# ErlerPhilipp/points2surf

Hardware: NVIDIA H100
Metric: SDF queries/sec at grid_res=256 (higher is better)
Workload: dtype f16 operands / f32 accumulate (wgmma); hi/lo split f16 (fp32-level) for FC tails and guard-band recompute

## Files before the change

points2surf_b200/csrc/net_tc.cu:

```cuda
#include "model.cuh"
#include "tc_ptx.cuh"

namespace p2s {

using namespace ptx;

namespace {

constexpr int kTile = 64;
constexpr int kWG = 2;
constexpr int kThreads = 128 * kWG;
template <bool PRECISE>
struct Cfg {
    static constexpr int kChunks = PRECISE ? 2 : 4;
    static constexpr int kSplit = 8 / kChunks;
    static constexpr uint32_t kChunkBytes = PRECISE ? 65536u : 32768u;
    static constexpr uint32_t kW3Bytes = kChunks * kChunkBytes;
    static constexpr uint32_t kMidScale = PRECISE ? 2u : 1u;
    static constexpr uint32_t kMidBytes = (8192u + 8192u + 16384u) * kMidScale;
    static constexpr uint32_t kPerqBytes = PRECISE ? 16384u : 8192u;
    static constexpr uint32_t kRedBytes = 4u * kChunks * 128u * 4u;
    static constexpr uint32_t kOffMid = kW3Bytes;
    static constexpr uint32_t kWgWq = kPerqBytes;
    static constexpr uint32_t kWgBytes = kWgWq + 192 * 4;
    static constexpr uint32_t kOffWg = kOffMid + kMidBytes;
    static constexpr uint32_t kOffBias = kOffWg + kWG * kWgBytes;
    static constexpr uint32_t kSmemBytes = kOffBias + 320 * 4;
};
static_assert(Cfg<false>::kSmemBytes <= 232448 && Cfg<true>::kSmemBytes <= 232448, "shared memory budget");
static_assert(Cfg<false>::kRedBytes <= Cfg<false>::kPerqBytes && Cfg<true>::kRedBytes <= Cfg<true>::kPerqBytes, "reduction scratch");

struct Seg {
    const float* ptr;
    int n;
    int tiles;
    int center;
};

struct PassParams {
    Seg seg[2];
    const float* query;
    const float* R;
    int tiles_per_query;
    int B;
    const float* W0;
    const float* b0;
    int num_mid;
    int mid_N[3];
    const uint8_t* mid_img[3];
    const float* mid_bias[3];
    int perq_layer;
    const uint8_t* perq_img;
    const uint8_t* w3_img;
    float* out;
};

__device__ __forceinline__ uint32_t pack_relu(float a, float b) {
    uint32_t r;
    asm("cvt.rn.relu.satfinite.f16x2.f32 %0, %1, %2;" : "=r"(r) : "f"(b), "f"(a));
    return r;
}
__device__ __forceinline__ void pack_relu_split(float a, float b, uint32_t& hi, uint32_t& lo) {
    hi = pack_relu(a, b);
    const float2 hf = __half22float2(*reinterpret_cast<const __half2*>(&hi));
    lo = pack_half2(fmaxf(a, 0.f) - hf.x, fmaxf(b, 0.f) - hf.y);
}
template <bool PRECISE>
__device__ __forceinline__ void pack_act(float a, float b, uint32_t& hi, uint32_t& lo) {
    if (PRECISE) pack_relu_split(a, b, hi, lo);
    else hi = pack_relu(a, b);
}

template <bool PRECISE, int R>
__device__ __forceinline__ void mid_mma(float (&d)[R], const uint32_t (&a)[4], const uint32_t (&al)[4], uint64_t w, uint64_t w_lo, uint32_t acc) {
    if (R == 32) {
        auto& d32 = reinterpret_cast<float (&)[32]>(d);
        if (PRECISE) { wgmma_rs_n64(d32, al, w, acc); wgmma_rs_n64(d32, a, w_lo, 1); wgmma_rs_n64(d32, a, w, 1); }
        else wgmma_rs_n64(d32, a, w, acc);
    } else {
        auto& d64 = reinterpret_cast<float (&)[64]>(d);
        if (PRECISE) { wgmma_rs_n128(d64, al, w, acc); wgmma_rs_n128(d64, a, w_lo, 1); wgmma_rs_n128(d64, a, w, 1); }
        else wgmma_rs_n128(d64, a, w, acc);
    }
}

template <bool PRECISE, int R, int KL>
__device__ __forceinline__ void pack_acc(const float (&d)[R], const float* bias, int q4, uint32_t (&a)[R / 8][4], uint32_t (&al)[R / 8][KL]) {
#pragma unroll
    for (int j = 0; j < R / 4; ++j) {
        const float2 bb = *reinterpret_cast<const float2*>(bias + 8 * j + 2 * q4);
        pack_act<PRECISE>(d[4 * j] + bb.x, d[4 * j + 1] + bb.y, a[j >> 1][(j & 1) * 2], al[j >> 1][PRECISE ? (j & 1) * 2 : 0]);
        pack_act<PRECISE>(d[4 * j + 2] + bb.x, d[4 * j + 3] + bb.y, a[j >> 1][(j & 1) * 2 + 1], al[j >> 1][PRECISE ? (j & 1) * 2 + 1 : 0]);
    }
}

template <int S>
__device__ __forceinline__ void max_halve(float (&m)[32], int lane) {
    const bool up = (lane & S) != 0;
#pragma unroll
    for (int i = 0; i < S; ++i) {
        const float send = up ? m[i] : m[i + S], keep = up ? m[i + S] : m[i];
        m[i] = fmaxf(keep, __shfl_xor_sync(0xffffffffu, send, S));
    }
}

template <bool PRECISE>
__global__ void __launch_bounds__(kThreads, 1) pointnet_pass_kernel(const PassParams p) {
    using C = Cfg<PRECISE>;
    constexpr int kL = PRECISE ? 4 : 1;
    extern __shared__ __align__(1024) uint8_t smem[];
    float* s_bias = reinterpret_cast<float*>(smem + C::kOffBias);
    const int tid = threadIdx.x, wg = tid >> 7, t = tid & 127, lane = tid & 31, q4 = lane & 3;
    const int r0 = (t >> 5) * 16 + (lane >> 2);
    const int part = blockIdx.x % C::kSplit;
    const int stream = blockIdx.x / C::kSplit, nstreams = gridDim.x / C::kSplit;
    const int nq = (p.B > stream) ? (p.B - stream + nstreams - 1) / nstreams : 0;
    const int tpq = p.tiles_per_query;
    uint32_t mid_off[3] = {0, 0, 0};
    {
        uint32_t o = 0;
        for (int l = 0; l < p.num_mid; ++l) { mid_off[l] = o; o += (uint32_t)p.mid_N[l] * 128u * C::kMidScale; }
    }

    if (nq > 0) {
        const uint4* src = reinterpret_cast<const uint4*>(p.w3_img + (size_t)part * C::kW3Bytes);
        uint4* dst = reinterpret_cast<uint4*>(smem);
        for (uint32_t i = tid; i < C::kW3Bytes / 16; i += kThreads) dst[i] = src[i];
        for (int l = 0; l < p.num_mid; ++l) {
            if (l == p.perq_layer) continue;
            const uint4* s = reinterpret_cast<const uint4*>(p.mid_img[l]);
            uint4* d = reinterpret_cast<uint4*>(smem + C::kOffMid + mid_off[l]);
            for (uint32_t i = tid; i < (uint32_t)p.mid_N[l] * 8u * C::kMidScale; i += kThreads) d[i] = s[i];
        }
    }
    {
        int off = 0;
        for (int l = 0; l < p.num_mid; ++l) {
            for (int i = tid; i < p.mid_N[l]; i += kThreads) s_bias[off + i] = p.mid_bias[l][i];
            off += p.mid_N[l];
        }
        for (int i = tid; i < 64; i += kThreads) s_bias[256 + i] = p.b0[i];
    }
    fence_proxy_async_smem();
    __syncthreads();

    uint8_t* wsm = smem + C::kOffWg + wg * C::kWgBytes;
    uint8_t* perq = wsm;
    float* red = reinterpret_cast<float*>(perq);
    float* wq = reinterpret_cast<float*>(wsm + C::kWgWq);
    const float* s_b0 = s_bias + 256;
    const uint32_t bar_id = 1 + (uint32_t)wg;
    auto wg_sync = [&]() { asm volatile("bar.sync %0, 128;" ::"r"(bar_id) : "memory"); };
    const uint64_t dsc_w3 = make_smem_desc(smem_u32(smem), 128, 2048);
    uint64_t dsc_mid[3], dsc_mid_lo[3];
    for (int l = 0; l < 3; ++l) {
        const bool pq = l == p.perq_layer;
        dsc_mid[l] = make_smem_desc(pq ? smem_u32(perq) : smem_u32(smem + C::kOffMid) + mid_off[l], 128, 1024);
        dsc_mid_lo[l] = dsc_mid[l] + (uint64_t)((pq ? 8192u : (uint32_t)p.mid_N[l] * 128u) >> 4);
    }

    for (int qi = wg; qi < nq; qi += kWG) {
        const size_t q = (size_t)stream + (size_t)qi * nstreams;
        wg_sync();
        if (t < 64) {
            const float w0 = p.W0[t * 3 + 0], w1 = p.W0[t * 3 + 1], w2 = p.W0[t * 3 + 2];
            float r[9] = {1.f, 0.f, 0.f, 0.f, 1.f, 0.f, 0.f, 0.f, 1.f};
            if (p.R) {
#pragma unroll
                for (int i = 0; i < 9; ++i) r[i] = p.R[q * 9 + i];
            }
            wq[0 * 64 + t] = w0 * r[0] + w1 * r[3] + w2 * r[6];
            wq[1 * 64 + t] = w0 * r[1] + w1 * r[4] + w2 * r[7];
            wq[2 * 64 + t] = w0 * r[2] + w1 * r[5] + w2 * r[8];
        }
        if (p.perq_layer >= 0) {
            const uint4* s = reinterpret_cast<const uint4*>(p.perq_img + q * C::kPerqBytes);
            uint4* d = reinterpret_cast<uint4*>(perq);
            for (uint32_t i = t; i < C::kPerqBytes / 16; i += 128) d[i] = s[i];
            fence_proxy_async_smem();
        }
        wg_sync();
        float vmax[4 * C::kChunks];
#pragma unroll
        for (int i = 0; i < 4 * C::kChunks; ++i) vmax[i] = -INFINITY;
        for (int tq = 0; tq < tpq; ++tq) {
            const int sgi = tq < p.seg[0].tiles ? 0 : 1;
            const Seg& sg = p.seg[sgi];
            float cx = 0.f, cy = 0.f, cz = 0.f;
            if (sg.center) { cx = p.query[q * 3 + 0]; cy = p.query[q * 3 + 1]; cz = p.query[q * 3 + 2]; }
            float px[2], py[2], pz[2];
#pragma unroll
            for (int h = 0; h < 2; ++h) {
                int local = (tq - (sgi ? p.seg[0].tiles : 0)) * kTile + r0 + 8 * h;
                if (local >= sg.n) local = 0;
                const float* src = sg.ptr + (q * sg.n + local) * 3;
                px[h] = src[0] - cx; py[h] = src[1] - cy; pz[h] = src[2] - cz;
            }
            uint32_t a[4][4], al[4][kL];
#pragma unroll
            for (int kk = 0; kk < 4; ++kk) {
#pragma unroll
                for (int hc = 0; hc < 2; ++hc) {
                    const int ch = kk * 16 + hc * 8 + 2 * q4;
                    const float2 wx = *reinterpret_cast<const float2*>(wq + 0 * 64 + ch);
                    const float2 wy = *reinterpret_cast<const float2*>(wq + 1 * 64 + ch);
                    const float2 wz = *reinterpret_cast<const float2*>(wq + 2 * 64 + ch);
                    const float2 bb = *reinterpret_cast<const float2*>(s_b0 + ch);
#pragma unroll
                    for (int h = 0; h < 2; ++h) {
                        const float v0 = fmaf(wx.x, px[h], fmaf(wy.x, py[h], fmaf(wz.x, pz[h], bb.x)));
                        const float v1 = fmaf(wx.y, px[h], fmaf(wy.y, py[h], fmaf(wz.y, pz[h], bb.y)));
                        pack_act<PRECISE>(v0, v1, a[kk][hc * 2 + h], al[kk][PRECISE ? hc * 2 + h : 0]);
                    }
                }
            }
            const float* bl = s_bias;
#pragma unroll
            for (int l = 0; l < 2; ++l) {
                if (l >= p.num_mid - 1) break;
                float d[32];
#pragma unroll
                for (int i = 0; i < 32; ++i) d[i] = 0.f;
                wgmma_fence();
#pragma unroll
                for (int ks = 0; ks < 4; ++ks)
                    mid_mma<PRECISE>(d, a[ks], reinterpret_cast<const uint32_t (&)[4]>(al[PRECISE ? ks : 0]), dsc_mid[l] + (uint64_t)(ks * 16), dsc_mid_lo[l] + (uint64_t)(ks * 16), ks > 0);
                wgmma_commit();
                wgmma_wait<0>();
                fence_regs(d);
                pack_acc<PRECISE>(d, bl, q4, a, al);
                bl += 64;
            }
            uint32_t a2[8][4], a2l[8][kL];
            {
                const uint64_t w = p.num_mid == 3 ? dsc_mid[2] : dsc_mid[0], w_lo = p.num_mid == 3 ? dsc_mid_lo[2] : dsc_mid_lo[0];
                float d[64];
#pragma unroll
                for (int i = 0; i < 64; ++i) d[i] = 0.f;
                wgmma_fence();
#pragma unroll
                for (int ks = 0; ks < 4; ++ks)
                    mid_mma<PRECISE>(d, a[ks], reinterpret_cast<const uint32_t (&)[4]>(al[PRECISE ? ks : 0]), w + (uint64_t)(ks * 16), w_lo + (uint64_t)(ks * 16), ks > 0);
                wgmma_commit();
                wgmma_wait<0>();
                fence_regs(d);
                pack_acc<PRECISE>(d, bl, q4, a2, a2l);
            }
#pragma unroll(PRECISE ? 1 : C::kChunks)
            for (int c = 0; c < C::kChunks; ++c) {
                float d[64];
#pragma unroll
                for (int i = 0; i < 64; ++i) d[i] = 0.f;
                const uint64_t w = dsc_w3 + (uint64_t)((uint32_t)c * (C::kChunkBytes >> 4));
                wgmma_fence();
#pragma unroll
                for (int ks = 0; ks < 8; ++ks) {
                    const uint64_t o = w + (uint64_t)(ks * 16);
                    if (PRECISE) {
                        wgmma_rs_n128(d, a2[ks], o + (uint64_t)(32768u >> 4), ks > 0);
                        wgmma_rs_n128(d, reinterpret_cast<const uint32_t (&)[4]>(a2l[PRECISE ? ks : 0]), o, 1);
                        wgmma_rs_n128(d, a2[ks], o, 1);
                    } else {
                        wgmma_rs_n128(d, a2[ks], o, ks > 0);
                    }
                }
                wgmma_commit();
                wgmma_wait<0>();
                fence_regs(d);
                float m[32];
#pragma unroll
                for (int j = 0; j < 16; ++j) {
                    m[2 * j] = fmaxf(d[4 * j], d[4 * j + 2]);
                    m[2 * j + 1] = fmaxf(d[4 * j + 1], d[4 * j + 3]);
                }
                max_halve<16>(m, lane);
                max_halve<8>(m, lane);
                max_halve<4>(m, lane);
                float v[4];
#pragma unroll
                for (int i = 0; i < 4; ++i) v[i] = fmaxf(vmax[i], m[i]);
#pragma unroll
                for (int i = 0; i < 4 * (C::kChunks - 1); ++i) vmax[i] = vmax[i + 4];
#pragma unroll
                for (int i = 0; i < 4; ++i) vmax[4 * (C::kChunks - 1) + i] = v[i];
            }
        }
        constexpr int kC = C::kChunks * 128;
        const int warp = t >> 5;
        wg_sync();
#pragma unroll
        for (int c = 0; c < C::kChunks; ++c)
#pragma unroll
            for (int h = 0; h < 2; ++h)
                *reinterpret_cast<float2*>(red + warp * kC + c * 128 + 16 * (lane >> 2) + 8 * h + 2 * q4) = make_float2(vmax[4 * c + 2 * h], vmax[4 * c + 2 * h + 1]);
        wg_sync();
        for (int i = t; i < kC / 4; i += 128) {
            const float4* r4 = reinterpret_cast<const float4*>(red);
            float4 v = r4[i];
#pragma unroll
            for (int w = 1; w < 4; ++w) {
                const float4 u = r4[w * (kC / 4) + i];
                v = make_float4(fmaxf(v.x, u.x), fmaxf(v.y, u.y), fmaxf(v.z, u.z), fmaxf(v.w, u.w));
            }
            *reinterpret_cast<float4*>(p.out + q * 1024 + (size_t)(part * kC + 4 * i)) = v;
        }
    }
}

__global__ void pack_kmajor_kernel(const float* __restrict__ W, int rows, int K, int row0, uint32_t sbo, uint8_t* __restrict__ img, int lo) {
    int e = blockIdx.x * blockDim.x + threadIdx.x;
    if (e >= rows * K) return;
    int r = e / K, k = e % K;
    uint32_t off = (uint32_t)(r >> 3) * sbo + (uint32_t)(k >> 3) * 128u + (uint32_t)(r & 7) * 16u + (uint32_t)(k & 7) * 2u;
    const float w = W[(size_t)(row0 + r) * K + k];
    const __half h = __float2half_rn(w);
    *reinterpret_cast<__half*>(img + off) = lo ? __float2half_rn(w - __half2float(h)) : h;
}

__global__ void pack_perq_kernel(const float* __restrict__ W, int64_t B, uint8_t* __restrict__ img) {
    int64_t e = (int64_t)blockIdx.x * blockDim.x + threadIdx.x;
    if (e >= B * 4096) return;
    int64_t b = e >> 12;
    int r = (int)((e >> 6) & 63), k = (int)(e & 63);
    uint32_t off = (uint32_t)(r >> 3) * 1024u + (uint32_t)(k >> 3) * 128u + (uint32_t)(r & 7) * 16u + (uint32_t)(k & 7) * 2u;
    *reinterpret_cast<__half*>(img + b * 8192 + off) = __float2half_rn(W[e]);
}

__global__ void __launch_bounds__(256) fold_w1_kernel(const float* __restrict__ W1, const float* __restrict__ T, int64_t B, uint8_t* __restrict__ img) {
    __shared__ float sW[64][65];
    __shared__ __align__(16) float sT[64][68];
    const int64_t b = blockIdx.x;
    const int tid = threadIdx.x;
    for (int e = tid; e < 4096; e += 256) {
        const int r = e >> 6, c = e & 63;
        sW[r][c] = W1[e];
        sT[r][c] = T[b * 4096 + e] + (r == c ? 1.0f : 0.0f);
    }
    __syncthreads();
    const int o = tid >> 2, i0 = (tid & 3) * 16;
    float acc[16];
#pragma unroll
    for (int i = 0; i < 16; ++i) acc[i] = 0.f;
    for (int j = 0; j < 64; ++j) {
        const float w = sW[o][j];
#pragma unroll
        for (int i4 = 0; i4 < 4; ++i4) {
            const float4 t4 = *reinterpret_cast<const float4*>(&sT[j][i0 + 4 * i4]);
            acc[4 * i4 + 0] = fmaf(w, t4.x, acc[4 * i4 + 0]);
            acc[4 * i4 + 1] = fmaf(w, t4.y, acc[4 * i4 + 1]);
            acc[4 * i4 + 2] = fmaf(w, t4.z, acc[4 * i4 + 2]);
            acc[4 * i4 + 3] = fmaf(w, t4.w, acc[4 * i4 + 3]);
        }
    }
    uint8_t* dst = img + b * 8192 + (uint32_t)(o >> 3) * 1024u + (uint32_t)(o & 7) * 16u;
#pragma unroll
    for (int h = 0; h < 2; ++h) {
        uint32_t v[4];
#pragma unroll
        for (int e = 0; e < 4; ++e) v[e] = pack_half2(acc[h * 8 + 2 * e], acc[h * 8 + 2 * e + 1]);
        *reinterpret_cast<uint4*>(dst + (uint32_t)(i0 / 8 + h) * 128u) = make_uint4(v[0], v[1], v[2], v[3]);
    }
}

__global__ void fold_fc3_kernel(const float* __restrict__ W1, const float* __restrict__ Wfc3, const float* __restrict__ bfc3,
                                float* __restrict__ G, float* __restrict__ g0) {
    const int oi = blockIdx.x;
    const int o = oi >> 6, i = oi & 63;
    const int k = threadIdx.x;
    float acc = 0.f;
    for (int j = 0; j < 64; ++j) acc = fmaf(W1[o * 64 + j], Wfc3[(size_t)(j * 64 + i) * 256 + k], acc);
    G[(size_t)oi * 256 + k] = acc;
    if (k == 0) {
        float b = W1[o * 64 + i];
        for (int j = 0; j < 64; ++j) b = fmaf(W1[o * 64 + j], bfc3[j * 64 + i], b);
        g0[oi] = b;
    }
}

__global__ void transpose64_kernel(const float* __restrict__ in, float* __restrict__ out, int64_t B) {
    int64_t e = (int64_t)blockIdx.x * blockDim.x + threadIdx.x;
    if (e >= B * 4096) return;
    int64_t b = e >> 12;
    int i = (int)((e >> 6) & 63), j = (int)(e & 63);
    out[e] = in[b * 4096 + j * 64 + i];
}

__global__ void guard_flag_kernel(const float* __restrict__ logits, int od, int64_t B, float band, int32_t* __restrict__ list, int* __restrict__ count, int64_t base, int64_t cap) {
    int64_t i = (int64_t)blockIdx.x * blockDim.x + threadIdx.x;
    if (i >= B) return;
    if (fabsf(logits[i * od + od - 1]) < band) {
        int slot = atomicAdd(count, 1);
        if (slot < cap) list[slot] = (int32_t)(base + i);
    }
}
__global__ void guard_gather_kernel(const float* __restrict__ src, const int32_t* __restrict__ list, int n, int row_floats, float* __restrict__ dst) {
    int64_t e = (int64_t)blockIdx.x * blockDim.x + threadIdx.x;
    if (e >= (int64_t)n * row_floats) return;
    int i = (int)(e / row_floats), j = (int)(e % row_floats);
    dst[e] = src[(int64_t)list[i] * row_floats + j];
}
__global__ void guard_scatter_kernel(const float* __restrict__ src, const int32_t* __restrict__ list, int n, int od, float* __restrict__ logits) {
    int i = blockIdx.x * blockDim.x + threadIdx.x;
    if (i >= n) return;
    for (int j = 0; j < od; ++j) logits[(int64_t)list[i] * od + j] = src[i * od + j];
}
__global__ void guard_scatter_rows_kernel(const float* __restrict__ src, const int32_t* __restrict__ list, int n, int row_floats, float* __restrict__ dst) {
    int64_t e = (int64_t)blockIdx.x * blockDim.x + threadIdx.x;
    if (e >= (int64_t)n * row_floats) return;
    int i = (int)(e / row_floats), j = (int)(e % row_floats);
    dst[(int64_t)list[i] * row_floats + j] = src[e];
}

}

struct TcStack {
    uint8_t* w3_img = nullptr;
    uint8_t* mid_img[3] = {nullptr, nullptr, nullptr};
    uint8_t* w3_img_p = nullptr;
    uint8_t* mid_img_p[3] = {nullptr, nullptr, nullptr};
    const float* mid_bias[3] = {nullptr, nullptr, nullptr};
    int mid_N[3] = {0, 0, 0};
    int num_mid = 0;
    const float* W0 = nullptr;
    const float* b0 = nullptr;
    const float* b3 = nullptr;
};

struct TcFc {
    const Layer* L = nullptr;
    const uint8_t* img = nullptr;
};
struct TcStnFc { TcFc fc1, fc2, fc3; };

struct TcWeights {
    TcStack qstn;
    TcStack stn[2], fin[2];
    TcStnFc qstn_fc, stn_fc[2];
    TcFc head_fc1[2], head_fc2, head_fc3;
    const uint8_t* fold_img[2] = {nullptr, nullptr};
    const float* fold_bias[2] = {nullptr, nullptr};
    TcStack stn_enc, fin_enc;
    TcStnFc stn_fc_enc;
    TcFc head_fc1_enc;
    const uint8_t* fold_img_enc = nullptr;
    const float* fold_bias_enc = nullptr;
    bool fc_on_tc = true;
    std::vector<void*> allocs;
    int sm_count = 132;
    bool prof_on = false;
    std::vector<std::pair<cudaEvent_t, cudaEvent_t>> prof_events;
    double prof_flops = 0.0;
    ~TcWeights() {
        for (void* a : allocs) cudaFree(a);
        for (auto& e : prof_events) { cudaEventDestroy(e.first); cudaEventDestroy(e.second); }
    }
};

namespace {

uint8_t* tc_alloc(TcWeights& t, size_t bytes) {
    void* p = nullptr;
    P2S_CUDA(cudaMalloc(&p, bytes));
    P2S_CUDA(cudaMemset(p, 0, bytes));
    t.allocs.push_back(p);
    return (uint8_t*)p;
}

uint8_t* pack_layer(TcWeights& t, const Layer& L, uint32_t sbo, bool split = false) {
    const size_t one = (size_t)L.cout * L.cin * 2;
    uint8_t* img = tc_alloc(t, one * (split ? 2 : 1));
    P2S_LAUNCH(pack_kmajor_kernel, (unsigned)cdiv((int64_t)L.cout * L.cin, 256), 256, 0, 0, L.W, L.cout, L.cin, 0, sbo, img, 0);
    if (split) P2S_LAUNCH(pack_kmajor_kernel, (unsigned)cdiv((int64_t)L.cout * L.cin, 256), 256, 0, 0, L.W, L.cout, L.cin, 0, sbo, img + one, 1);
    return img;
}

uint8_t* pack_w3(TcWeights& t, const Layer& L, bool split = false) {
    P2S_CHECK(L.cout == 1024 && L.cin == 128, "big layer must be 128 -> 1024");
    const size_t chunk = split ? 65536 : 32768;
    uint8_t* img = tc_alloc(t, 8 * chunk);
    for (int c = 0; c < 8; ++c) {
        P2S_LAUNCH(pack_kmajor_kernel, (unsigned)cdiv(128 * 128, 256), 256, 0, 0, L.W, 128, 128, c * 128, 2048u, img + (size_t)c * chunk, 0);
        if (split) P2S_LAUNCH(pack_kmajor_kernel, (unsigned)cdiv(128 * 128, 256), 256, 0, 0, L.W, 128, 128, c * 128, 2048u, img + (size_t)c * chunk + 32768, 1);
    }
    return img;
}

void launch_pass(Model& m, const TcStack& s, const Seg& s0, const Seg& s1, const float* query, const float* R,
                 int64_t B, int perq_layer, const uint8_t* perq_img, float* out, cudaStream_t st, bool precise) {
    PassParams p{};
    p.seg[0] = s0; p.seg[1] = s1;
    p.query = query; p.R = R;
    p.tiles_per_query = s0.tiles + s1.tiles;
    p.B = (int)B;
    p.W0 = s.W0; p.b0 = s.b0;
    p.num_mid = s.num_mid;
    for (int l = 0; l < 3; ++l) { p.mid_N[l] = s.mid_N[l]; p.mid_img[l] = precise ? s.mid_img_p[l] : s.mid_img[l]; p.mid_bias[l] = s.mid_bias[l]; }
    p.perq_layer = perq_layer;
    p.perq_img = perq_img;
    p.w3_img = precise ? s.w3_img_p : s.w3_img;
    p.out = out;
    for (int l = 0; l < s.num_mid; ++l)
        P2S_CHECK(s.mid_N[l] == (l == s.num_mid - 1 ? 128 : 64), "pass kernel: mid layers must be 64 -> 64 ... -> 128");
    TcWeights& t = *m.tc;
    const int split = precise ? Cfg<true>::kSplit : Cfg<false>::kSplit;
    int streams = t.sm_count / split;
    if ((int64_t)streams > B) streams = (int)B;
    const int grid = streams * split;
    cudaEvent_t e0 = nullptr, e1 = nullptr;
    const bool prof = t.prof_on && !precise;
    if (prof) {
        P2S_CUDA(cudaEventCreate(&e0)); P2S_CUDA(cudaEventCreate(&e1));
        P2S_CUDA(cudaEventRecord(e0, st));
    }
    if (precise) P2S_LAUNCH(pointnet_pass_kernel<true>, grid, kThreads, Cfg<true>::kSmemBytes, st, p);
    else P2S_LAUNCH(pointnet_pass_kernel<false>, grid, kThreads, Cfg<false>::kSmemBytes, st, p);
    if (prof) {
        P2S_CUDA(cudaEventRecord(e1, st));
        t.prof_events.emplace_back(e0, e1);
        double mac_pt = 3.0 * 64 + 128.0 * 1024;
        int prev = 64;
        for (int l = 0; l < s.num_mid; ++l) { mac_pt += (double)prev * s.mid_N[l]; prev = s.mid_N[l]; }
        t.prof_flops += 2.0 * mac_pt * (double)(s0.n + s1.n) * (double)B;
    }
}

Seg make_seg(const float* ptr, int n, int center) { return Seg{ptr, n, n > 0 ? (n + kTile - 1) / kTile : 0, center}; }

void run_fc(const TcFc& f, const float* in, int lda, float* out, int ldc, int64_t Bc, bool relu, bool on_tc, cudaStream_t st,
            const float* in_bias = nullptr, bool in_relu = false) {
    const Layer& L = *f.L;
    if (on_tc && f.img) launch_fc_tc(in, lda, f.img, L.b, out, ldc, Bc, L.cout, L.cin, relu, st, 0, in_bias, in_relu);
    else {
        P2S_CHECK(!in_bias, "input bias needs the tensor-core FC kernel");
        launch_gemm_nt(in, 0, lda, L.W, 0, L.b, out, 0, ldc, (int)Bc, L.cout, L.cin, 1, relu, st);
    }
}

void fc_tail(const Layer& b3src, const TcStnFc& s, bool on_tc, const float* gmax_raw, int64_t Bc, float* g, float* f1, float* f2, float* out, cudaStream_t st) {
    if (on_tc && s.fc1.img) run_fc(s.fc1, gmax_raw, 1024, f1, 512, Bc, true, true, st, b3src.b, true);
    else {
        P2S_CUDA(cudaMemcpyAsync(g, gmax_raw, (size_t)Bc * 1024 * 4, cudaMemcpyDeviceToDevice, st));
        launch_bias_act(g, b3src.b, Bc, 1024, true, st);
        run_fc(s.fc1, g, 1024, f1, 512, Bc, true, on_tc, st);
    }
    run_fc(s.fc2, f1, 512, f2, 256, Bc, true, on_tc, st);
    run_fc(s.fc3, f2, 256, out, s.fc3.L->cout, Bc, false, on_tc, st);
}

}

void tc_build(Model& m) {
    P2S_CHECK(m.cfg.net_size == 1024, "tensor-core path needs net_size 1024");
    TcWeights* t = new TcWeights();
    m.tc = t;
    cudaDeviceProp prop;
    P2S_CUDA(cudaGetDeviceProperties(&prop, m.device));
    t->sm_count = prop.multiProcessorCount;
    P2S_CUDA(cudaFuncSetAttribute(pointnet_pass_kernel<false>, cudaFuncAttributeMaxDynamicSharedMemorySize, (int)Cfg<false>::kSmemBytes));
    P2S_CUDA(cudaFuncSetAttribute(pointnet_pass_kernel<true>, cudaFuncAttributeMaxDynamicSharedMemorySize, (int)Cfg<true>::kSmemBytes));
    auto build_stn = [&](TcStack& s, const Stn& stn, const Layer* c0a, const Layer* c0b) {
        if (!c0a) {
            s.W0 = stn.c1.W; s.b0 = stn.c1.b;
            s.num_mid = 1;
            s.mid_img[0] = pack_layer(*t, stn.c2, 1024); s.mid_bias[0] = stn.c2.b; s.mid_N[0] = 128;
            s.mid_img_p[0] = pack_layer(*t, stn.c2, 1024, true);
        } else {
            s.W0 = c0a->W; s.b0 = c0a->b;
            s.num_mid = 3;
            s.mid_img[0] = pack_layer(*t, *c0b, 1024); s.mid_bias[0] = c0b->b; s.mid_N[0] = 64;
            s.mid_img[1] = pack_layer(*t, stn.c1, 1024); s.mid_bias[1] = stn.c1.b; s.mid_N[1] = 64;
            s.mid_img[2] = pack_layer(*t, stn.c2, 1024); s.mid_bias[2] = stn.c2.b; s.mid_N[2] = 128;
            s.mid_img_p[0] = pack_layer(*t, *c0b, 1024, true);
            s.mid_img_p[1] = pack_layer(*t, stn.c1, 1024, true);
            s.mid_img_p[2] = pack_layer(*t, stn.c2, 1024, true);
        }
        s.w3_img_p = pack_w3(*t, stn.c3, true);
        s.w3_img = pack_w3(*t, stn.c3);
        s.b3 = stn.c3.b;
    };
    auto build_fin = [&](TcStack& s, const Feat& f) {
        s.W0 = f.conv0a.W; s.b0 = f.conv0a.b;
        s.num_mid = 3;
        s.mid_img[0] = pack_layer(*t, f.conv0b, 1024); s.mid_bias[0] = f.conv0b.b; s.mid_N[0] = 64;
        s.mid_img[1] = nullptr; s.mid_bias[1] = f.conv1.b; s.mid_N[1] = 64;
        s.mid_img[2] = pack_layer(*t, f.conv2, 1024); s.mid_bias[2] = f.conv2.b; s.mid_N[2] = 128;
        s.mid_img_p[0] = pack_layer(*t, f.conv0b, 1024, true);
        s.mid_img_p[2] = pack_layer(*t, f.conv2, 1024, true);
        s.w3_img_p = pack_w3(*t, f.conv3, true);
        s.w3_img = pack_w3(*t, f.conv3);
        s.b3 = f.conv3.b;
    };
    fc_tc_init();
    t->fc_on_tc = !env_flag("P2S_FC_FP32");
    auto mk_fc = [&](const Layer& L) {
        TcFc f;
        f.L = &L;
        f.img = fc_tc_supported(L.cout, L.cin) ? fc_tc_pack(L, t->allocs) : nullptr;
        return f;
    };
    auto mk_stn_fc = [&](const Stn& s) { TcStnFc r; r.fc1 = mk_fc(s.fc1); r.fc2 = mk_fc(s.fc2); r.fc3 = mk_fc(s.fc3); return r; };
    auto fold = [&](const Feat& f, const uint8_t*& img, const float*& bias) {
        P2S_CHECK(f.stn2.fc3.cout == 4096 && f.stn2.fc3.cin == 256 && f.conv1.cout == 64 && f.conv1.cin == 64, "unexpected STN shape");
        float* G = reinterpret_cast<float*>(tc_alloc(*t, (size_t)4096 * 256 * 4));
        float* g0 = reinterpret_cast<float*>(tc_alloc(*t, 4096 * 4));
        P2S_LAUNCH(fold_fc3_kernel, 4096, 256, 0, 0, f.conv1.W, f.stn2.fc3.W, f.stn2.fc3.b, G, g0);
        img = fc_tc_pack_raw(G, 4096, 256, t->allocs);
        bias = g0;
    };
    if (m.single_transformer) {
        t->qstn_fc = mk_stn_fc(m.enc.stn1);
        t->stn_fc_enc = mk_stn_fc(m.enc.stn2);
        fold(m.enc, t->fold_img_enc, t->fold_bias_enc);
        t->head_fc1_enc = mk_fc(m.fc1_enc);
        t->head_fc2 = mk_fc(m.fc2);
        t->head_fc3 = mk_fc(m.fc3);
        build_stn(t->qstn, m.enc.stn1, nullptr, nullptr);
        build_stn(t->stn_enc, m.enc.stn2, &m.enc.conv0a, &m.enc.conv0b);
        build_fin(t->fin_enc, m.enc);
        P2S_CUDA(cudaDeviceSynchronize());
        return;
    }
    if (m.shared_qstn) t->qstn_fc = mk_stn_fc(m.point_stn);
    else if (m.global.has_qstn) t->qstn_fc = mk_stn_fc(m.global.stn1);
    t->stn_fc[0] = mk_stn_fc(m.local.stn2);
    t->stn_fc[1] = mk_stn_fc(m.global.stn2);
    for (int br = 0; br < 2; ++br) fold(br ? m.global : m.local, t->fold_img[br], t->fold_bias[br]);
    t->head_fc1[0] = mk_fc(m.fc1_local);
    t->head_fc1[1] = mk_fc(m.fc1_global);
    t->head_fc2 = mk_fc(m.fc2);
    t->head_fc3 = mk_fc(m.fc3);
    if (m.shared_qstn) build_stn(t->qstn, m.point_stn, nullptr, nullptr);
    else if (m.global.has_qstn) build_stn(t->qstn, m.global.stn1, nullptr, nullptr);
    build_stn(t->stn[0], m.local.stn2, &m.local.conv0a, &m.local.conv0b);
    build_stn(t->stn[1], m.global.stn2, &m.global.conv0a, &m.global.conv0b);
    build_fin(t->fin[0], m.local);
    build_fin(t->fin[1], m.global);
    P2S_CUDA(cudaDeviceSynchronize());
}

void tc_destroy(Model& m) {
    delete m.tc;
    m.tc = nullptr;
}

void tc_profile_reset(Model& m, bool on) {
    TcWeights& t = *m.tc;
    for (auto& e : t.prof_events) { cudaEventDestroy(e.first); cudaEventDestroy(e.second); }
    t.prof_events.clear();
    t.prof_flops = 0.0;
    t.prof_on = on;
}

void tc_profile_get(Model& m, double* ms, int64_t* launches, double* flops) {
    TcWeights& t = *m.tc;
    double total = 0.0;
    for (auto& e : t.prof_events) {
        P2S_CUDA(cudaEventSynchronize(e.second));
        float x = 0.f;
        P2S_CUDA(cudaEventElapsedTime(&x, e.first, e.second));
        total += x;
    }
    *ms = total;
    *launches = (int64_t)t.prof_events.size();
    *flops = t.prof_flops;
}

static void forward_tc_core(Model& m, const float* patch, const float* sub, const float* query, int64_t B,
                            float* logits, cudaStream_t st, bool precise) {
    TcWeights& t = *m.tc;
    const int P = m.cfg.points_per_patch, S = m.cfg.sub_sample_size;
    const int64_t Bc_max = 8192;
    const size_t per_q = 1024 * 4 + 512 + 256 + 4 + 9 + 4096 * 2 + 1024 + 256 + 128 + 4096  + 16 +
                         1024 + 512 + 256 ;
    float* base = m.ws_net.as<float>(per_q * (size_t)Bc_max + 1024);
    float* pcur = base;
    auto take = [&](size_t n) { float* r = pcur; pcur += (n * (size_t)Bc_max + 63) / 64 * 64; return r; };
    float* gmax = take(1024); float* g = take(1024); float* f1 = take(512); float* f2 = take(256);
    float* q4 = take(4); float* R = take(9); float* T = take(4096); float* Tt = take(4096);
    float* fmax_l = take(1024); float* fmax_g = take(1024); float* cat = take(1024); float* h3 = take(256); float* h4 = take(128);
    uint8_t* perq = reinterpret_cast<uint8_t*>(take(4096));
    uint8_t* imgA = reinterpret_cast<uint8_t*>(take(1024)); uint8_t* imgB = reinterpret_cast<uint8_t*>(take(512)); uint8_t* imgC = reinterpret_cast<uint8_t*>(take(256));
    const bool fc_tc = t.fc_on_tc || precise;
    auto img_ok = [](const TcStnFc& f) { return f.fc1.img && f.fc2.img; };
    auto stn_tail_img = [&](const Layer& c3, const TcStnFc& f, const float* gmax_raw, int64_t Bc, float* out_f2) {
        launch_pack_a(gmax_raw, 1024, Bc, 1024, c3.b, true, imgA, st);
        launch_fc_tc_img(imgA, f.fc1.img, f.fc1.L->b, imgB, 0, Bc, 512, 1024, true, st, 3, 16, 0);
        if (out_f2) launch_fc_tc_img(imgB, f.fc2.img, f.fc2.L->b, out_f2, 256, Bc, 256, 512, true, st, 0);
        else launch_fc_tc_img(imgB, f.fc2.img, f.fc2.L->b, imgC, 0, Bc, 256, 512, true, st, 3, 8, 0);
    };
    auto qstn_rot = [&](const Layer& c3, int64_t Bc) {
        { StageScope ts("net: fc tails", st);
          if (fc_tc && img_ok(t.qstn_fc)) {
              stn_tail_img(c3, t.qstn_fc, gmax, Bc, f2);
              run_fc(t.qstn_fc.fc3, f2, 256, q4, 4, Bc, false, false, st);
          } else fc_tail(c3, t.qstn_fc, fc_tc, gmax, Bc, g, f1, f2, q4, st); }
        launch_quat_to_rot(q4, R, Bc, st);
    };
    auto stn64_perq = [&](const Feat& f, const TcStnFc& fc, const uint8_t* fold_img, const float* fold_bias, int64_t Bc) {
        if (fc_tc) {
            StageScope ts("net: fc tails", st);
            if (img_ok(fc)) {
                stn_tail_img(f.stn2.c3, fc, gmax, Bc, nullptr);
                launch_fc_tc_img(imgC, fold_img, fold_bias, perq, 0, Bc, 4096, 256, false, st, precise ? 2 : 1);
            } else {
                run_fc(fc.fc1, gmax, 1024, f1, 512, Bc, true, true, st, f.stn2.c3.b, true);
                run_fc(fc.fc2, f1, 512, f2, 256, Bc, true, true, st);
                launch_fc_tc(f2, 256, fold_img, fold_bias, reinterpret_cast<float*>(perq), 0, Bc, 4096, 256, false, st, precise ? 2 : 1);
            }
        } else {
            { StageScope ts("net: fc tails", st); fc_tail(f.stn2.c3, fc, false, gmax, Bc, g, f1, f2, T, st); }
            { StageScope ts("net: fold W1*T", st); P2S_LAUNCH(fold_w1_kernel, (unsigned)Bc, 256, 0, st, f.conv1.W, T, Bc, perq); }
        }
// ... 127 lines not shown
```

points2surf_b200/csrc/tc_ptx.cuh:

```cuda
#pragma once
#include <cstdint>
#include <cuda_fp16.h>

namespace p2s {
namespace ptx {

__device__ __forceinline__ uint32_t smem_u32(const void* p) { return (uint32_t)__cvta_generic_to_shared(p); }

__device__ __forceinline__ void mbar_init(uint64_t* bar, uint32_t count) {
    asm volatile("mbarrier.init.shared::cta.b64 [%0], %1;" ::"r"(smem_u32(bar)), "r"(count) : "memory");
}
__device__ __forceinline__ void fence_mbar_init() { asm volatile("fence.mbarrier_init.release.cluster;" ::: "memory"); }
__device__ __forceinline__ void mbar_arrive(uint64_t* bar) {
    asm volatile("mbarrier.arrive.shared::cta.b64 _, [%0];" ::"r"(smem_u32(bar)) : "memory");
}
__device__ __forceinline__ void mbar_arrive_expect_tx(uint64_t* bar, uint32_t bytes) {
    asm volatile("mbarrier.arrive.expect_tx.shared::cta.b64 _, [%0], %1;" ::"r"(smem_u32(bar)), "r"(bytes) : "memory");
}
__device__ __forceinline__ bool mbar_try_wait(uint64_t* bar, uint32_t parity) {
    uint32_t ok;
    asm volatile(
        "{\n\t.reg .pred p;\n\t"
        "mbarrier.try_wait.parity.shared::cta.b64 p, [%1], %2;\n\t"
        "selp.u32 %0, 1, 0, p;\n\t}"
        : "=r"(ok) : "r"(smem_u32(bar)), "r"(parity) : "memory");
    return ok != 0;
}
__device__ __forceinline__ void mbar_wait_bounded(uint64_t* bar, uint32_t parity) {
    long long t0 = clock64();
    while (!mbar_try_wait(bar, parity)) {
        if (clock64() - t0 > 2000000000LL) __trap();
    }
}
__device__ __forceinline__ bool mbar_test_wait(uint64_t* bar, uint32_t parity) {
    uint32_t ok;
    asm volatile(
        "{\n\t.reg .pred p;\n\t"
        "mbarrier.test_wait.parity.shared::cta.b64 p, [%1], %2;\n\t"
        "selp.u32 %0, 1, 0, p;\n\t}"
        : "=r"(ok) : "r"(smem_u32(bar)), "r"(parity) : "memory");
    return ok != 0;
}
__device__ __forceinline__ void mbar_wait(uint64_t* bar, uint32_t parity) {
    while (!mbar_try_wait(bar, parity)) {}
}

__device__ __forceinline__ bool elect_one() {
    uint32_t pred;
    asm volatile("{\n\t.reg .pred P1;\n\telect.sync _|P1, 0xffffffff;\n\tselp.u32 %0, 1, 0, P1;\n\t}" : "=r"(pred));
    return pred != 0;
}

__device__ __forceinline__ void fence_proxy_async_smem() { asm volatile("fence.proxy.async.shared::cta;" ::: "memory"); }

__device__ __forceinline__ void bulk_g2s(void* smem_dst, const void* gmem_src, uint32_t bytes, uint64_t* bar) {
    asm volatile("cp.async.bulk.shared::cluster.global.mbarrier::complete_tx::bytes [%0], [%1], %2, [%3];"
                 ::"r"(smem_u32(smem_dst)), "l"(gmem_src), "r"(bytes), "r"(smem_u32(bar)) : "memory");
}

__device__ __forceinline__ uint64_t make_smem_desc(uint32_t smem_addr, uint32_t lbo_bytes, uint32_t sbo_bytes) {
    uint64_t d = 0;
    d |= (uint64_t)((smem_addr & 0x3FFFFu) >> 4);
    d |= (uint64_t)((lbo_bytes >> 4) & 0x3FFFu) << 16;
    d |= (uint64_t)((sbo_bytes >> 4) & 0x3FFFu) << 32;
    return d;
}

__device__ __forceinline__ void wgmma_fence() { asm volatile("wgmma.fence.sync.aligned;" ::: "memory"); }
__device__ __forceinline__ void wgmma_commit() { asm volatile("wgmma.commit_group.sync.aligned;" ::: "memory"); }
template <int N>
__device__ __forceinline__ void wgmma_wait() { asm volatile("wgmma.wait_group.sync.aligned %0;" ::"n"(N) : "memory"); }
template <int R>
__device__ __forceinline__ void fence_regs(float (&d)[R]) {
#pragma unroll
    for (int i = 0; i < R; ++i) asm volatile("" : "+f"(d[i])::"memory");
}
__device__ __forceinline__ void wgmma_rs_n64(float (&d)[32], const uint32_t (&a)[4], uint64_t b_desc, uint32_t accumulate) {
    asm volatile(
        "{\n\t.reg .pred p;\n\tsetp.ne.b32 p, %37, 0;\n\t"
        "wgmma.mma_async.sync.aligned.m64n64k16.f32.f16.f16 {%0, %1, %2, %3, %4, %5, %6, %7, %8, %9, %10, %11, %12, %13, %14, %15, %16, %17, %18, %19, %20, %21, %22, %23, %24, %25, %26, %27, %28, %29, %30, %31}, {%32, %33, %34, %35}, %36, p, 1, 1, 0;\n\t}"
        : "+f"(d[0]), "+f"(d[1]), "+f"(d[2]), "+f"(d[3]), "+f"(d[4]), "+f"(d[5]), "+f"(d[6]), "+f"(d[7]), "+f"(d[8]), "+f"(d[9]), "+f"(d[10]), "+f"(d[11]), "+f"(d[12]), "+f"(d[13]), "+f"(d[14]), "+f"(d[15]), "+f"(d[16]), "+f"(d[17]), "+f"(d[18]), "+f"(d[19]), "+f"(d[20]), "+f"(d[21]), "+f"(d[22]), "+f"(d[23]), "+f"(d[24]), "+f"(d[25]), "+f"(d[26]), "+f"(d[27]), "+f"(d[28]), "+f"(d[29]), "+f"(d[30]), "+f"(d[31])
        : "r"(a[0]), "r"(a[1]), "r"(a[2]), "r"(a[3]), "l"(b_desc), "r"(accumulate) : "memory");
}
__device__ __forceinline__ void wgmma_rs_n128(float (&d)[64], const uint32_t (&a)[4], uint64_t b_desc, uint32_t accumulate) {
    asm volatile(
        "{\n\t.reg .pred p;\n\tsetp.ne.b32 p, %69, 0;\n\t"
        "wgmma.mma_async.sync.aligned.m64n128k16.f32.f16.f16 {%0, %1, %2, %3, %4, %5, %6, %7, %8, %9, %10, %11, %12, %13, %14, %15, %16, %17, %18, %19, %20, %21, %22, %23, %24, %25, %26, %27, %28, %29, %30, %31, %32, %33, %34, %35, %36, %37, %38, %39, %40, %41, %42, %43, %44, %45, %46, %47, %48, %49, %50, %51, %52, %53, %54, %55, %56, %57, %58, %59, %60, %61, %62, %63}, {%64, %65, %66, %67}, %68, p, 1, 1, 0;\n\t}"
        : "+f"(d[0]), "+f"(d[1]), "+f"(d[2]), "+f"(d[3]), "+f"(d[4]), "+f"(d[5]), "+f"(d[6]), "+f"(d[7]), "+f"(d[8]), "+f"(d[9]), "+f"(d[10]), "+f"(d[11]), "+f"(d[12]), "+f"(d[13]), "+f"(d[14]), "+f"(d[15]), "+f"(d[16]), "+f"(d[17]), "+f"(d[18]), "+f"(d[19]), "+f"(d[20]), "+f"(d[21]), "+f"(d[22]), "+f"(d[23]), "+f"(d[24]), "+f"(d[25]), "+f"(d[26]), "+f"(d[27]), "+f"(d[28]), "+f"(d[29]), "+f"(d[30]), "+f"(d[31]), "+f"(d[32]), "+f"(d[33]), "+f"(d[34]), "+f"(d[35]), "+f"(d[36]), "+f"(d[37]), "+f"(d[38]), "+f"(d[39]), "+f"(d[40]), "+f"(d[41]), "+f"(d[42]), "+f"(d[43]), "+f"(d[44]), "+f"(d[45]), "+f"(d[46]), "+f"(d[47]), "+f"(d[48]), "+f"(d[49]), "+f"(d[50]), "+f"(d[51]), "+f"(d[52]), "+f"(d[53]), "+f"(d[54]), "+f"(d[55]), "+f"(d[56]), "+f"(d[57]), "+f"(d[58]), "+f"(d[59]), "+f"(d[60]), "+f"(d[61]), "+f"(d[62]), "+f"(d[63])
        : "r"(a[0]), "r"(a[1]), "r"(a[2]), "r"(a[3]), "l"(b_desc), "r"(accumulate) : "memory");
}
__device__ __forceinline__ void wgmma_ss_n128(float (&d)[64], uint64_t a_desc, uint64_t b_desc, uint32_t accumulate) {
    asm volatile(
        "{\n\t.reg .pred p;\n\tsetp.ne.b32 p, %66, 0;\n\t"
        "wgmma.mma_async.sync.aligned.m64n128k16.f32.f16.f16 {%0, %1, %2, %3, %4, %5, %6, %7, %8, %9, %10, %11, %12, %13, %14, %15, %16, %17, %18, %19, %20, %21, %22, %23, %24, %25, %26, %27, %28, %29, %30, %31, %32, %33, %34, %35, %36, %37, %38, %39, %40, %41, %42, %43, %44, %45, %46, %47, %48, %49, %50, %51, %52, %53, %54, %55, %56, %57, %58, %59, %60, %61, %62, %63}, %64, %65, p, 1, 1, 0, 0;\n\t}"
        : "+f"(d[0]), "+f"(d[1]), "+f"(d[2]), "+f"(d[3]), "+f"(d[4]), "+f"(d[5]), "+f"(d[6]), "+f"(d[7]), "+f"(d[8]), "+f"(d[9]), "+f"(d[10]), "+f"(d[11]), "+f"(d[12]), "+f"(d[13]), "+f"(d[14]), "+f"(d[15]), "+f"(d[16]), "+f"(d[17]), "+f"(d[18]), "+f"(d[19]), "+f"(d[20]), "+f"(d[21]), "+f"(d[22]), "+f"(d[23]), "+f"(d[24]), "+f"(d[25]), "+f"(d[26]), "+f"(d[27]), "+f"(d[28]), "+f"(d[29]), "+f"(d[30]), "+f"(d[31]), "+f"(d[32]), "+f"(d[33]), "+f"(d[34]), "+f"(d[35]), "+f"(d[36]), "+f"(d[37]), "+f"(d[38]), "+f"(d[39]), "+f"(d[40]), "+f"(d[41]), "+f"(d[42]), "+f"(d[43]), "+f"(d[44]), "+f"(d[45]), "+f"(d[46]), "+f"(d[47]), "+f"(d[48]), "+f"(d[49]), "+f"(d[50]), "+f"(d[51]), "+f"(d[52]), "+f"(d[53]), "+f"(d[54]), "+f"(d[55]), "+f"(d[56]), "+f"(d[57]), "+f"(d[58]), "+f"(d[59]), "+f"(d[60]), "+f"(d[61]), "+f"(d[62]), "+f"(d[63])
        : "l"(a_desc), "l"(b_desc), "r"(accumulate) : "memory");
}

__device__ __forceinline__ uint32_t pack_half2(float lo, float hi) {
    __half2 h = __floats2half2_rn(lo, hi);
    return *reinterpret_cast<uint32_t*>(&h);
}

}
}
```

Before: 421,000.

## Share per-tile layer-3 activations across a 2-CTA cluster via DSMEM

In the fast path, the two CTAs that split the final-layer output channels now run as a cluster of two. Each CTA computes the early point-MLP layers for only every other tile and pushes the resulting 128-wide activations into its peer's shared memory with st.async and mbarriers. Previously both CTAs recomputed the same front layers, so this halves that redundant work. In exchange it adds cross-CTA synchronization, extra shared-memory slots, a cluster launch that may reduce the number of concurrent streams, and a risk of stalls when the two peers drift out of step.

```diff
diff --git a/points2surf_b200/csrc/net_tc.cu b/points2surf_b200/csrc/net_tc.cu
--- a/points2surf_b200/csrc/net_tc.cu
+++ b/points2surf_b200/csrc/net_tc.cu
@@ -25,7 +25,10 @@
     static constexpr uint32_t kWgBytes = kWgWq + 192 * 4;
     static constexpr uint32_t kOffWg = kOffMid + kMidBytes;
     static constexpr uint32_t kOffBias = kOffWg + kWG * kWgBytes;
-    static constexpr uint32_t kSmemBytes = kOffBias + 320 * 4;
+    static constexpr uint32_t kSlotBytes = PRECISE ? 0u : 8u * 128u * 16u;
+    static constexpr uint32_t kOffSlot = kOffBias + 320 * 4;
+    static constexpr uint32_t kOffXBar = kOffSlot + kWG * kSlotBytes;
+    static constexpr uint32_t kSmemBytes = kOffXBar + (PRECISE ? 0u : kWG * 16u);
 };
 static_assert(Cfg<false>::kSmemBytes <= 232448 && Cfg<true>::kSmemBytes <= 232448, "shared memory budget");
 static_assert(Cfg<false>::kRedBytes <= Cfg<false>::kPerqBytes && Cfg<true>::kRedBytes <= Cfg<true>::kPerqBytes, "reduction scratch");
@@ -119,14 +122,18 @@
     uint32_t mid_off[3] = {0, 0, 0};
     {
         uint32_t o = 0;
-        for (int l = 0; l < p.num_mid; ++l) { mid_off[l] = o; o += (uint32_t)p.mid_N[l] * 128u * C::kMidScale; }
+        for (int l = 0; l < (PRECISE ? p.num_mid : 3); ++l) {
+            if (!PRECISE && l >= p.num_mid) break;
+            mid_off[l] = o; o += (uint32_t)p.mid_N[l] * 128u * C::kMidScale;
+        }
     }
 
     if (nq > 0) {
         const uint4* src = reinterpret_cast<const uint4*>(p.w3_img + (size_t)part * C::kW3Bytes);
         uint4* dst = reinterpret_cast<uint4*>(smem);
         for (uint32_t i = tid; i < C::kW3Bytes / 16; i += kThreads) dst[i] = src[i];
-        for (int l = 0; l < p.num_mid; ++l) {
+        for (int l = 0; l < (PRECISE ? p.num_mid : 3); ++l) {
+            if (!PRECISE && l >= p.num_mid) break;
             if (l == p.perq_layer) continue;
             const uint4* s = reinterpret_cast<const uint4*>(p.mid_img[l]);
             uint4* d = reinterpret_cast<uint4*>(smem + C::kOffMid + mid_off[l]);
@@ -141,8 +148,18 @@
         }
         for (int i = tid; i < 64; i += kThreads) s_bias[256 + i] = p.b0[i];
     }
+    uint64_t* xbar = reinterpret_cast<uint64_t*>(smem + C::kOffXBar);
+    if (!PRECISE && tid == 0) {
+        for (int w = 0; w < kWG; ++w) {
+            mbar_init(xbar + 2 * w, 1);
+            mbar_arrive_expect_tx(xbar + 2 * w, C::kSlotBytes);
+            mbar_init(xbar + 2 * w + 1, 128);
+        }
+        fence_mbar_init();
+    }
     fence_proxy_async_smem();
     __syncthreads();
+    if (!PRECISE) cluster_sync();
 
     uint8_t* wsm = smem + C::kOffWg + wg * C::kWgBytes;
     uint8_t* perq = wsm;
@@ -158,6 +175,11 @@
         dsc_mid[l] = make_smem_desc(pq ? smem_u32(perq) : smem_u32(smem + C::kOffMid) + mid_off[l], 128, 1024);
         dsc_mid_lo[l] = dsc_mid[l] + (uint64_t)((pq ? 8192u : (uint32_t)p.mid_N[l] * 128u) >> 4);
     }
+    uint8_t* slot = smem + C::kOffSlot + wg * C::kSlotBytes;
+    uint64_t* full = xbar + 2 * wg;
+    uint64_t* empty = xbar + 2 * wg + 1;
+    const uint32_t peer = (uint32_t)part ^ 1u;
+    uint32_t nsend = 0, nrecv = 0;
 
     for (int qi = wg; qi < nq; qi += kWG) {
         const size_t q = (size_t)stream + (size_t)qi * nstreams;
@@ -183,68 +205,90 @@
         float vmax[4 * C::kChunks];
 #pragma unroll
         for (int i = 0; i < 4 * C::kChunks; ++i) vmax[i] = -INFINITY;
-        for (int tq = 0; tq < tpq; ++tq) {
-            const int sgi = tq < p.seg[0].tiles ? 0 : 1;
-            const Seg& sg = p.seg[sgi];
-            float cx = 0.f, cy = 0.f, cz = 0.f;
-            if (sg.center) { cx = p.query[q * 3 + 0]; cy = p.query[q * 3 + 1]; cz = p.query[q * 3 + 2]; }
-            float px[2], py[2], pz[2];
-#pragma unroll
-            for (int h = 0; h < 2; ++h) {
-                int local = (tq - (sgi ? p.seg[0].tiles : 0)) * kTile + r0 + 8 * h;
-                if (local >= sg.n) local = 0;
-                const float* src = sg.ptr + (q * sg.n + local) * 3;
-                px[h] = src[0] - cx; py[h] = src[1] - cy; pz[h] = src[2] - cz;
-            }
-            uint32_t a[4][4], al[4][kL];
-#pragma unroll
-            for (int kk = 0; kk < 4; ++kk) {
-#pragma unroll
-                for (int hc = 0; hc < 2; ++hc) {
-                    const int ch = kk * 16 + hc * 8 + 2 * q4;
-                    const float2 wx = *reinterpret_cast<const float2*>(wq + 0 * 64 + ch);
-                    const float2 wy = *reinterpret_cast<const float2*>(wq + 1 * 64 + ch);
-                    const float2 wz = *reinterpret_cast<const float2*>(wq + 2 * 64 + ch);
-                    const float2 bb = *reinterpret_cast<const float2*>(s_b0 + ch);
-#pragma unroll
-                    for (int h = 0; h < 2; ++h) {
-                        const float v0 = fmaf(wx.x, px[h], fmaf(wy.x, py[h], fmaf(wz.x, pz[h], bb.x)));
-                        const float v1 = fmaf(wx.y, px[h], fmaf(wy.y, py[h], fmaf(wz.y, pz[h], bb.y)));
-                        pack_act<PRECISE>(v0, v1, a[kk][hc * 2 + h], al[kk][PRECISE ? hc * 2 + h : 0]);
+        const int own = PRECISE ? 0 : (part ^ wg ^ (qi >> 1)) & 1;
+        for (int i = 0; i < tpq; ++i) {
+            const int tq = PRECISE ? i : (i & ~1) + own;
+            const bool mine = PRECISE || (!(i & 1) && tq < tpq);
+            uint32_t a2[8][4], a2l[8][kL];
+            if (mine) {
+                const int sgi = tq < p.seg[0].tiles ? 0 : 1;
+                const Seg& sg = p.seg[sgi];
+                float cx = 0.f, cy = 0.f, cz = 0.f;
+                if (sg.center) { cx = p.query[q * 3 + 0]; cy = p.query[q * 3 + 1]; cz = p.query[q * 3 + 2]; }
+                float px[2], py[2], pz[2];
+#pragma unroll
+                for (int h = 0; h < 2; ++h) {
+                    int local = (tq - (sgi ? p.seg[0].tiles : 0)) * kTile + r0 + 8 * h;
+                    if (local >= sg.n) local = 0;
+                    const float* src = sg.ptr + (q * sg.n + local) * 3;
+                    px[h] = src[0] - cx; py[h] = src[1] - cy; pz[h] = src[2] - cz;
+                }
+                uint32_t a[4][4], al[4][kL];
+#pragma unroll
+                for (int kk = 0; kk < 4; ++kk) {
+#pragma unroll
+                    for (int hc = 0; hc < 2; ++hc) {
+                        const int ch = kk * 16 + hc * 8 + 2 * q4;
+                        const float2 wx = *reinterpret_cast<const float2*>(wq + 0 * 64 + ch);
+                        const float2 wy = *reinterpret_cast<const float2*>(wq + 1 * 64 + ch);
+                        const float2 wz = *reinterpret_cast<const float2*>(wq + 2 * 64 + ch);
+                        const float2 bb = *reinterpret_cast<const float2*>(s_b0 + ch);
+#pragma unroll
+                        for (int h = 0; h < 2; ++h) {
+                            const float v0 = fmaf(wx.x, px[h], fmaf(wy.x, py[h], fmaf(wz.x, pz[h], bb.x)));
+                            const float v1 = fmaf(wx.y, px[h], fmaf(wy.y, py[h], fmaf(wz.y, pz[h], bb.y)));
+                            pack_act<PRECISE>(v0, v1, a[kk][hc * 2 + h], al[kk][PRECISE ? hc * 2 + h : 0]);
+                        }
                     }
                 }
-            }
-            const float* bl = s_bias;
-#pragma unroll
-            for (int l = 0; l < 2; ++l) {
-                if (l >= p.num_mid - 1) break;
-                float d[32];
-#pragma unroll
-                for (int i = 0; i < 32; ++i) d[i] = 0.f;
-                wgmma_fence();
-#pragma unroll
-                for (int ks = 0; ks < 4; ++ks)
-                    mid_mma<PRECISE>(d, a[ks], reinterpret_cast<const uint32_t (&)[4]>(al[PRECISE ? ks : 0]), dsc_mid[l] + (uint64_t)(ks * 16), dsc_mid_lo[l] + (uint64_t)(ks * 16), ks > 0);
-                wgmma_commit();
-                wgmma_wait<0>();
-                fence_regs(d);
-                pack_acc<PRECISE>(d, bl, q4, a, al);
-                bl += 64;
-            }
-            uint32_t a2[8][4], a2l[8][kL];
-            {
-                const uint64_t w = p.num_mid == 3 ? dsc_mid[2] : dsc_mid[0], w_lo = p.num_mid == 3 ? dsc_mid_lo[2] : dsc_mid_lo[0];
-                float d[64];
-#pragma unroll
-                for (int i = 0; i < 64; ++i) d[i] = 0.f;
-                wgmma_fence();
-#pragma unroll
-                for (int ks = 0; ks < 4; ++ks)
-                    mid_mma<PRECISE>(d, a[ks], reinterpret_cast<const uint32_t (&)[4]>(al[PRECISE ? ks : 0]), w + (uint64_t)(ks * 16), w_lo + (uint64_t)(ks * 16), ks > 0);
-                wgmma_commit();
-                wgmma_wait<0>();
-                fence_regs(d);
-                pack_acc<PRECISE>(d, bl, q4, a2, a2l);
+                const float* bl = s_bias;
+#pragma unroll
+                for (int l = 0; l < 2; ++l) {
+                    if (l >= p.num_mid - 1) break;
+                    float d[32];
+#pragma unroll
+                    for (int i = 0; i < 32; ++i) d[i] = 0.f;
+                    wgmma_fence();
+#pragma unroll
+                    for (int ks = 0; ks < 4; ++ks)
+                        mid_mma<PRECISE>(d, a[ks], reinterpret_cast<const uint32_t (&)[4]>(al[PRECISE ? ks : 0]), dsc_mid[l] + (uint64_t)(ks * 16), dsc_mid_lo[l] + (uint64_t)(ks * 16), ks > 0);
+                    wgmma_commit();
+                    wgmma_wait<0>();
+                    fence_regs(d);
+                    pack_acc<PRECISE>(d, bl, q4, a, al);
+                    bl += 64;
+                }
+                {
+                    const uint64_t w = p.num_mid == 3 ? dsc_mid[2] : dsc_mid[0], w_lo = p.num_mid == 3 ? dsc_mid_lo[2] : dsc_mid_lo[0];
+                    float d[64];
+#pragma unroll
+                    for (int i = 0; i < 64; ++i) d[i] = 0.f;
+                    wgmma_fence();
+#pragma unroll
+                    for (int ks = 0; ks < 4; ++ks)
+                        mid_mma<PRECISE>(d, a[ks], reinterpret_cast<const uint32_t (&)[4]>(al[PRECISE ? ks : 0]), w + (uint64_t)(ks * 16), w_lo + (uint64_t)(ks * 16), ks > 0);
+                    wgmma_commit();
+                    wgmma_wait<0>();
+                    fence_regs(d);
+                    pack_acc<PRECISE>(d, bl, q4, a2, a2l);
+                }
+                if (!PRECISE) {
+                    if (nsend > 0) mbar_wait_cluster_bounded(empty, (nsend - 1) & 1);
+                    const uint32_t dst = mapa(smem_u32(slot), peer) + 16u * (uint32_t)t, bar = mapa(smem_u32(full), peer);
+#pragma unroll
+                    for (int k = 0; k < 8; ++k) st_async_v4(dst + 2048u * k, a2[k], bar);
+                    ++nsend;
+                }
+            } else {
+                mbar_wait_cluster_bounded(full, nrecv & 1);
+#pragma unroll
+                for (int k = 0; k < 8; ++k) {
+                    const uint4 v = reinterpret_cast<const uint4*>(slot)[128 * k + t];
+                    a2[k][0] = v.x; a2[k][1] = v.y; a2[k][2] = v.z; a2[k][3] = v.w;
+                }
+                mbar_arrive_cluster(mapa(smem_u32(empty), peer));
+                if (t == 0) mbar_arrive_expect_tx(full, C::kSlotBytes);
+                ++nrecv;
             }
 #pragma unroll(PRECISE ? 1 : C::kChunks)
             for (int c = 0; c < C::kChunks; ++c) {
@@ -305,6 +349,7 @@
             *reinterpret_cast<float4*>(p.out + q * 1024 + (size_t)(part * kC + 4 * i)) = v;
         }
     }
+    if (!PRECISE) cluster_sync();
 }
 
 __global__ void pack_kmajor_kernel(const float* __restrict__ W, int rows, int K, int row0, uint32_t sbo, uint8_t* __restrict__ img, int lo) {
@@ -447,6 +492,7 @@
     bool fc_on_tc = true;
     std::vector<void*> allocs;
     int sm_count = 132;
+    int pass_clusters = 66;
     bool prof_on = false;
     std::vector<std::pair<cudaEvent_t, cudaEvent_t>> prof_events;
     double prof_flops = 0.0;
@@ -483,6 +529,21 @@
         if (split) P2S_LAUNCH(pack_kmajor_kernel, (unsigned)cdiv(128 * 128, 256), 256, 0, 0, L.W, 128, 128, c * 128, 2048u, img + (size_t)c * chunk + 32768, 1);
     }
     return img;
+}
+
+cudaLaunchConfig_t pass_cluster_config(int grid, cudaStream_t st, cudaLaunchAttribute (&attr)[1]) {
+    cudaLaunchConfig_t cfg{};
+    cfg.gridDim = dim3((unsigned)grid);
+    cfg.blockDim = dim3(kThreads);
+    cfg.dynamicSmemBytes = Cfg<false>::kSmemBytes;
+    cfg.stream = st;
+    attr[0].id = cudaLaunchAttributeClusterDimension;
+    attr[0].val.clusterDim.x = 2;
+    attr[0].val.clusterDim.y = 1;
+    attr[0].val.clusterDim.z = 1;
+    cfg.attrs = attr;
+    cfg.numAttrs = 1;
+    return cfg;
 }
 
 void launch_pass(Model& m, const TcStack& s, const Seg& s0, const Seg& s1, const float* query, const float* R,
@@ -503,7 +564,7 @@
         P2S_CHECK(s.mid_N[l] == (l == s.num_mid - 1 ? 128 : 64), "pass kernel: mid layers must be 64 -> 64 ... -> 128");
     TcWeights& t = *m.tc;
     const int split = precise ? Cfg<true>::kSplit : Cfg<false>::kSplit;
-    int streams = t.sm_count / split;
+    int streams = precise ? t.sm_count / split : t.pass_clusters;
     if ((int64_t)streams > B) streams = (int)B;
     const int grid = streams * split;
     cudaEvent_t e0 = nullptr, e1 = nullptr;
@@ -513,7 +574,12 @@
         P2S_CUDA(cudaEventRecord(e0, st));
     }
     if (precise) P2S_LAUNCH(pointnet_pass_kernel<true>, grid, kThreads, Cfg<true>::kSmemBytes, st, p);
-    else P2S_LAUNCH(pointnet_pass_kernel<false>, grid, kThreads, Cfg<false>::kSmemBytes, st, p);
+    else {
+        cudaLaunchAttribute cluster[1];
+        const cudaLaunchConfig_t cfg = pass_cluster_config(grid, st, cluster);
+        P2S_CUDA(cudaLaunchKernelEx(&cfg, pointnet_pass_kernel<false>, p));
+        g_launches.fetch_add(1, std::memory_order_relaxed);
+    }
     if (prof) {
         P2S_CUDA(cudaEventRecord(e1, st));
         t.prof_events.emplace_back(e0, e1);
@@ -558,6 +624,14 @@
     t->sm_count = prop.multiProcessorCount;
     P2S_CUDA(cudaFuncSetAttribute(pointnet_pass_kernel<false>, cudaFuncAttributeMaxDynamicSharedMemorySize, (int)Cfg<false>::kSmemBytes));
     P2S_CUDA(cudaFuncSetAttribute(pointnet_pass_kernel<true>, cudaFuncAttributeMaxDynamicSharedMemorySize, (int)Cfg<true>::kSmemBytes));
+    {
+        cudaLaunchAttribute cluster[1];
+        const cudaLaunchConfig_t cfg = pass_cluster_config(2 * (t->sm_count / 2), 0, cluster);
+        int clusters = 0;
+        P2S_CUDA(cudaOccupancyMaxActiveClusters(&clusters, pointnet_pass_kernel<false>, &cfg));
+        P2S_CHECK(clusters > 0, "pass kernel: no cluster of two CTAs fits on the device");
+        t->pass_clusters = std::min(clusters, t->sm_count / 2);
+    }
     auto build_stn = [&](TcStack& s, const Stn& stn, const Layer* c0a, const Layer* c0b) {
         if (!c0a) {
             s.W0 = stn.c1.W; s.b0 = stn.c1.b;
diff --git a/points2surf_b200/csrc/tc_ptx.cuh b/points2surf_b200/csrc/tc_ptx.cuh
--- a/points2surf_b200/csrc/tc_ptx.cuh
+++ b/points2surf_b200/csrc/tc_ptx.cuh
@@ -43,6 +43,37 @@
 }
 __device__ __forceinline__ void mbar_wait(uint64_t* bar, uint32_t parity) {
     while (!mbar_try_wait(bar, parity)) {}
+}
+
+__device__ __forceinline__ uint32_t mapa(uint32_t addr, uint32_t rank) {
+    uint32_t r;
+    asm("mapa.shared::cluster.u32 %0, %1, %2;" : "=r"(r) : "r"(addr), "r"(rank));
+    return r;
+}
+__device__ __forceinline__ void cluster_sync() {
+    asm volatile("barrier.cluster.arrive.release;\n\tbarrier.cluster.wait.acquire;" ::: "memory");
+}
+__device__ __forceinline__ void st_async_v4(uint32_t addr, const uint32_t (&v)[4], uint32_t bar_addr) {
+    asm volatile("st.async.shared::cluster.mbarrier::complete_tx::bytes.v4.b32 [%0], {%1, %2, %3, %4}, [%5];"
+                 ::"r"(addr), "r"(v[0]), "r"(v[1]), "r"(v[2]), "r"(v[3]), "r"(bar_addr) : "memory");
+}
+__device__ __forceinline__ void mbar_arrive_cluster(uint32_t bar_addr) {
+    asm volatile("mbarrier.arrive.release.cluster.shared::cluster.b64 _, [%0];" ::"r"(bar_addr) : "memory");
+}
+__device__ __forceinline__ bool mbar_try_wait_cluster(uint64_t* bar, uint32_t parity) {
+    uint32_t ok;
+    asm volatile(
+        "{\n\t.reg .pred p;\n\t"
+        "mbarrier.try_wait.parity.acquire.cluster.shared::cta.b64 p, [%1], %2;\n\t"
+        "selp.u32 %0, 1, 0, p;\n\t}"
+        : "=r"(ok) : "r"(smem_u32(bar)), "r"(parity) : "memory");
+    return ok != 0;
+}
+__device__ __forceinline__ void mbar_wait_cluster_bounded(uint64_t* bar, uint32_t parity) {
+    long long t0 = clock64();
+    while (!mbar_try_wait_cluster(bar, parity)) {
+        if (clock64() - t0 > 2000000000LL) __trap();
+    }
 }
 
 __device__ __forceinline__ bool elect_one() {
```

Result: faster. 433,900, median of 6 (+3.1%).
